# batd-htplus/intool-rag

Hardware: AMD Instinct MI355X
Metric: queries/sec, exact top-10 inner-product search, 1M x 1024-d fp32 index (higher is better)
Workload: dtype bf16 x bf16 -> f32 filter scan, f64 re-score of the f32 rows; 1 GPU; configs[1]: 1M x 1024-d synthetic unit vectors, brute-force inner-product top-10; rows=1000000, dim=1024, k=10, queries_per_pass=64, exchange=none, steps_in_flight=4, world=1, backend=none, allgather_payload_bytes_per_rank=0

## Files before the change

include/hiprag.h:

```cpp
#ifndef HIPRAG_H
#define HIPRAG_H

#include <stdint.h>

#ifdef __cplusplus
extern "C" {
#endif

#define HIPRAG_OK 0
#define HIPRAG_E_INVALID (-1)
#define HIPRAG_E_HIP (-2)
#define HIPRAG_E_HANDLE (-3)
#define HIPRAG_E_IO (-4)
#define HIPRAG_E_NOMEM (-5)
#define HIPRAG_E_UNSUPPORTED (-6)

#define HIPRAG_METRIC_IP 0
#define HIPRAG_METRIC_L2 1

int32_t hiprag_version(void);
const char* hiprag_last_error(void);
int32_t hiprag_device_count(int32_t* out_count);
int32_t hiprag_device_sync(int32_t device);
int32_t hiprag_scan_stream(int32_t device, void** out_stream);
// ... 54 lines not shown
    int32_t wide_env;
    int32_t n_cu;
    int32_t launch_env;
} hipidx_scan_shape_t;
typedef struct hipidx_scan_plan_t {
    int32_t run;
    int32_t wide;
    int32_t waves;
    int32_t ring;
    int32_t multi_pass;
    int32_t filter;
    int32_t ncls;
    int32_t qtile_image;
    int64_t lds_bytes;
    int32_t launch_queries;
    int32_t pipe_spare_cus;
    int64_t bytes_per_pass_ip;
    int64_t bytes_per_pass_l2;
} hipidx_scan_plan_t;
int32_t hiprag_scan_plan(const hipidx_scan_shape_t* shape, int32_t nq, int32_t k, int32_t cus, hipidx_scan_plan_t* out);
int32_t hipidx_scan_shape(uint64_t h, hipidx_scan_shape_t* out);
int32_t hiprag_wide_walk(int64_t nrt, int32_t ncol, int32_t cus, int32_t wg, int64_t cap, int64_t* out_row_tile,
                         int32_t* out_column, int64_t* out_pairs);
int32_t hipidx_gate_tail_dev(uint64_t h, int32_t slot, void* stream);
int32_t hipidx_reserve_search(uint64_t h, int32_t k);
int32_t hipidx_reserve_rows(uint64_t h, int64_t n_rows);
int32_t hipidx_reconstruct(uint64_t h, int64_t row, float* out_host);
int32_t hipidx_save(uint64_t h, const char* path);
int32_t hipidx_load(const char* path, int32_t device, uint64_t* out_handle);

typedef struct hipidx_stats {
    int64_t passes;
    int64_t queries;
    int64_t fallback_queries;
    int64_t bytes_per_pass;
    int64_t timed_passes;
    float avg_scan_ms;
    float avg_scan_wall_ms;
    float avg_scan_gap_ms;
    int64_t launches;
    int64_t roundb_queries;
    int64_t list_entries;
    int64_t ranked_entries;
    int64_t rescored_groups;
    int64_t wide_launches;
} hipidx_stats;
int32_t hipidx_get_stats(uint64_t h, hipidx_stats* out);
int32_t hipidx_enable_timing(uint64_t h, int32_t on);

int32_t hipivf_create(uint64_t rows_h, uint64_t centroids_h, const int64_t* list_offsets_host, const int64_t* orig_ids_host,
                      int32_t nlist, uint64_t* out_handle);
int32_t hipivf_destroy(uint64_t h);
int32_t hipivf_search_dev(uint64_t h, const float* q_dev, int32_t nq, int32_t k, int32_t nprobe, double* out_scores64_dev,
                          float* out_scores_dev, int64_t* out_ids_dev, void* stream);
int32_t hipivf_info(uint64_t h, int32_t* out_nlist, int64_t* out_stored_rows, int64_t* out_longest_list);
int32_t hipivf_search_batch_dev(uint64_t h, const float* q_dev, int32_t nq, int32_t k, int32_t nprobe,
                                double* out_scores64_dev, float* out_scores_dev, int64_t* out_ids_dev, void* stream);
int32_t hipivf_batch_info(uint64_t h, int64_t* out4);
int32_t hipivf_search_scoped_dev(uint64_t h, const float* q_dev, int32_t nq, int32_t k, int32_t nprobe,
                                 const int64_t* ranges_host, const int32_t* scope_offsets_host, int32_t n_scopes,
                                 const int32_t* scope_of_query_host, double* out_scores64_dev, float* out_scores_dev,
                                 int64_t* out_ids_dev, void* stream);
int32_t hipivf_search_scoped(uint64_t h, const float* q_host, int32_t nq, int32_t k, int32_t nprobe,
                             const int64_t* ranges_host, const int32_t* scope_offsets_host, int32_t n_scopes,
                             const int32_t* scope_of_query_host, double* out_scores64, float* out_scores, int64_t* out_ids);
int32_t hipivf_scoped_info(uint64_t h, int64_t* out4);
#define HIPIVF_PROBE_ANY   0
#define HIPIVF_PROBE_SCOPE 1
// ... 319 lines not shown
```

intool-rag_amd/csrc/dense_api.hip:

```cpp
#include <cstring>
#include <vector>

#include "common.h"
#include "dense_internal.h"

namespace hiprag {

Registry<DenseIndex>& reg()
{
    static Registry<DenseIndex> r;
    return r;
}

int32_t create_dense(int32_t d, int32_t metric, int32_t device, std::shared_ptr<DenseIndex>& out)
{
    HR_REQUIRE(d > 0, "d must be positive (got %d)", d);
    HR_REQUIRE(metric == HIPRAG_METRIC_IP || metric == HIPRAG_METRIC_L2, "unknown metric %d", metric);
    const int P = ((d + 127) / 128) * 16;
    if ((size_t)P * 1024 > 128 * 1024) {
        set_error("d=%d needs %d KiB of LDS for the query tile; the scan supports d <= 1024 (128 KiB, leaving 32 KiB per CU "
                  "for the tail kernels of earlier passes)", d, P);
        return HIPRAG_E_UNSUPPORTED;
    }
    auto ix = std::make_shared<DenseIndex>();
// ... 306 lines not shown

int32_t hipidx_get_stats(uint64_t h, hipidx_stats* out)
{
    GET_INDEX(h);
    HR_REQUIRE(out, "null out");
    HR_CHECK_HIP(hipDeviceSynchronize());
    unsigned long long fb = 0;
    HR_CHECK_HIP(hipMemcpy(&fb, ix->fallback_counter(), sizeof(fb), hipMemcpyDeviceToHost));
    out->passes = ix->passes;
    out->launches = ix->launches;
    out->queries = ix->queries;
    out->fallback_queries = (int64_t)fb;
    {
        unsigned long long rbq = 0;
        HR_CHECK_HIP(hipMemcpy(&rbq, ix->extend_counter(), sizeof(rbq), hipMemcpyDeviceToHost));
        out->roundb_queries = (int64_t)rbq;
        unsigned long long wc[3] = {0, 0, 0};
        HR_CHECK_HIP(hipMemcpy(wc, ix->work_counters(), sizeof(wc), hipMemcpyDeviceToHost));
        out->list_entries = (int64_t)wc[0];
        out->ranked_entries = (int64_t)wc[1];
        out->rescored_groups = (int64_t)wc[2];
    }
    out->wide_launches = ix->wide_launches;
    out->bytes_per_pass = bytes_per_pass(ix->shape(), ix->metric, ix->wide_launch(ix->launch_q));
    return ix->timing.summarise(ix->nblocks() > 0, out);
}

}
```

intool-rag_amd/csrc/dense_index.hip:

```cpp
#include <atomic>
#include <cfloat>
#include <cmath>
#include <chrono>
#include <cstring>
#include <vector>

#include "common.h"
#include "topk_device.h"
#include "dense_internal.h"

namespace hiprag {
namespace {

__global__ void retile_kernel(const float* __restrict__ src, int64_t row0, int64_t n, int d, int P,
                              float4* __restrict__ xb)
{
    const int64_t blk0 = row0 / kRowsPerBlock;
    const int64_t nblk = (row0 + n - 1) / kRowsPerBlock - blk0 + 1;
    const int64_t t = (int64_t)blockIdx.x * blockDim.x + threadIdx.x;
    if (t >= nblk * P * kPieceVec4) return;
    const int lane = (int)(t & 63);
    const int64_t pp = t >> 6;
    const int p = (int)(pp % P);
    const int64_t blk = blk0 + pp / P;
// ... 117 lines not shown
        if (pipe_done[i]) (void)hipEventDestroy(pipe_done[i]);
    }
    if (add_ev) (void)hipEventDestroy(add_ev);
    for (hipEvent_t e : sc.pin_ev) if (e) (void)hipEventDestroy(e);
}

int32_t DenseIndex::init()
{
    HR_CHECK_HIP(hipSetDevice(device));
    hipDeviceProp_t prop;
    HR_CHECK_HIP(hipGetDeviceProperties(&prop, device));
    n_cu = prop.multiProcessorCount > 0 ? prop.multiProcessorCount : 256;
    scan_cus = n_cu;
    if (const char* ms = getenv("HIPRAG_SCAN_MODE")) {
        if (!strcmp(ms, "bf16")) scan_mode = kScanBf16;
        else if (!strcmp(ms, "q64")) scan_mode = kScanQ64;
        else { set_error("HIPRAG_SCAN_MODE=%s: the scan has two operand modes, bf16 (default) and q64", ms); return HIPRAG_E_INVALID; }
    }
    if (const char* sw = getenv("HIPRAG_SCAN_WIDE")) {
        if (!strcmp(sw, "0")) scan_wide = 0;
        else if (!strcmp(sw, "1")) scan_wide = 1;
        else { set_error("HIPRAG_SCAN_WIDE=%s: 0 (never the wide scan kernel) or 1 (whenever a launch is eligible)", sw); return HIPRAG_E_INVALID; }
    }
    const char* lq = getenv("HIPRAG_LAUNCH_QUERIES");
    launch_env = lq ? atoi(lq) : 0;
    update_launch_q();
    int32_t rc = scalars.reserve(64);
    if (rc) return rc;
    if ((rc = started.reserve(256))) return rc;
    HR_CHECK_HIP(hipMemset(started.p, 0, 256));
    gate = started.as<unsigned long long>() + 16;
    HR_CHECK_HIP(hipMemset(scalars.p, 0, 64));
    HR_CHECK_HIP(hipStreamSynchronize(nullptr));
    return HIPRAG_OK;
}

int32_t DenseIndex::grow(int64_t need_blocks)
{
    if (need_blocks <= cap_blocks) return HIPRAG_OK;
    {
        const int32_t wrc = wait_adds_host();
        if (wrc) return wrc;
    }
    int64_t nc = cap_blocks == 0 ? need_blocks : std::max(need_blocks, cap_blocks + cap_blocks / 2);
    size_t xbytes = (size_t)nc * P * kPieceFloats * sizeof(float);
    size_t nbytes = (size_t)nc * kRowsPerBlock * sizeof(float);
// ... 174 lines not shown

template <int METRIC>
int32_t DenseIndex::scan_pass(const float* q_dev, int nq, int k, int slot, int cus, hipStream_t st)
{
    Workspace& w = ws[slot];
    const ScanPlan pl = plan(nq, k, cus);
    const bool use_ev = timing.bracket() && pl.run;
    w.seq = 0;
    if (pl.run) {
        if (w.dirty) HR_CHECK_HIP(hipMemsetAsync(w.state.p, 0, w.state.bytes, st));
        w.dirty = true;
        w.waves = pl.waves;
        ScanArgs sa;
        sa.xb = xb.as<float4>(); sa.xh = xh.p; sa.q = q_dev; sa.norms = norms.as<float>();
        sa.slots = st_slots(w); sa.thetac = st_thetac(w); sa.count = st_count(w);
        sa.list = w.list.as<Cand>();
        sa.nblocks = nblocks(); sa.ntotal = ntotal; sa.nq = nq; sa.d = d; sa.P = P;
        sa.filter = pl.filter ? 1 : 0;
        sa.ncls = pl.ncls;
        sa.stamps = timing.launch_stamps();
        w.seq = ++scan_seq;
        started_total += (unsigned long long)cus;
        sa.started = started.as<unsigned long long>(); sa.target = started_total; sa.seq = w.seq; sa.gate = gate;
        sa.qtile = nullptr;
        if (pl.qtile_image) {
            const int npass = (nq + kPassQ - 1) / kPassQ, per_pass = P * 64;
            hipLaunchKernelGGL(qtile_kernel, dim3((unsigned)((per_pass + 255) / 256), (unsigned)npass), dim3(256), 0, st, q_dev, nq, d,
                               P / 2, w.qtile.as<bf16x8>());
            sa.qtile = w.qtile.p;
        }
        const ScanKernel scan = scan_kernel_of<METRIC>(pl, scan_mode);
        if (pl.wide) ++wide_launches;
        { int32_t lrc = ensure_lds(reinterpret_cast<const void*>(scan), pl.lds_bytes); if (lrc) return lrc; }
        if (use_ev) HR_CHECK_HIP(hipEventRecord(timing.edge(0), st));
        hipLaunchKernelGGL(scan, dim3(cus), dim3(pl.waves * 64), pl.lds_bytes, st, sa);
        if (use_ev) HR_CHECK_HIP(hipEventRecord(timing.edge(1), st));
    }
    w.ev_idx = timing.note(use_ev, pl.run ? cus * w.waves : 0);
    HR_CHECK_HIP(hipGetLastError());
    passes += (nq + kPassQ - 1) / kPassQ;
    ++launches;
    queries += nq;
    return HIPRAG_OK;
}

template <int METRIC>
// ... 207 lines not shown
```

intool-rag_amd/csrc/dense_internal.h:

```cpp
#pragma once
#include <atomic>
#include <vector>

#include "common.h"
#include "dense_layout.h"
#include "dense_plan.h"

namespace hiprag {

struct GroupWorkspace {
    DevBuf tiles, len, offs, chunks, order, items, stat, ps, pi;
    i64 chunk = 0, chunks_n = 0;
};

struct ScanTiming {
    static constexpr int kEvRing = 512;
    static constexpr int kMaxScanWaves = 12;
    bool on = false;
    int every = 1;
    int64_t count = 0;
    std::vector<hipEvent_t> evs;
    DevBuf stamps;
    int n_cu = 0, wall_khz = 100000;
    std::vector<char> ev_set;
// ... 2 lines not shown
    ~ScanTiming() { for (hipEvent_t e : evs) (void)hipEventDestroy(e); }
    void enable(int n) { on = n != 0; every = std::max(1, n); count = 0; }
    int32_t ensure(int n_cu_, int device);
    int slot() const { return (int)(count % kEvRing); }
    bool bracket() const { return on && count % every == 0; }
    unsigned long long* launch_stamps() const
    {
        return on ? stamps.as<unsigned long long>() + (size_t)slot() * n_cu * kMaxScanWaves * 2 : nullptr;
    }
    hipEvent_t edge(int which) const { return evs[2 * slot() + which]; }
    int note(bool bracketed, int waves);
    int32_t summarise(bool have_rows, hipidx_stats* out) const;
};

struct DenseIndex {
    std::mutex mu;
    int device = 0;
    int d = 0, P = 0, metric = 0;
    int64_t ntotal = 0, cap_blocks = 0, id_base = 0;
    int n_cu = 256;
    int scan_cus = 256;
    ScanMode scan_mode = kScanBf16;
    int scan_wide = -1;
    DevBuf xb, xh, norms, scalars;
    struct Workspace {
        DevBuf list, state, flags, ek, ei;
        DevBuf qtile;
        int k = 0, q = 0;
        int64_t blocks = 0;
        int ev_idx = -1;
        bool dirty = false;
        int waves = 8;
        unsigned long long seq = 0;
    };
    static constexpr int kSlots = 8;
    Workspace ws[kSlots];
    DevBuf qbuf, o64, o32, oid;
    struct Scoped {
        static constexpr int kRing = 4;
        PinBuf pin[kRing];
        hipEvent_t pin_ev[kRing] = {nullptr, nullptr, nullptr, nullptr};
        bool pin_used[kRing] = {false, false, false, false};
        int pin_next = 0;
        DevBuf meta;
        GroupWorkspace gw;
        int32_t upload(const int64_t* img, size_t words, hipStream_t st);
    } sc;
    DevBuf score_stat;
    i64 score_pairs = 0;
    PinBuf pin_q, pin_o32, pin_oid, pin_flags;
    unsigned long long* gate = nullptr;
    DevBuf started;
    unsigned long long scan_seq = 0, started_total = 0;
    static constexpr int kFewQueries = 16;
    int launch_q = 256;
    int launch_env = 0;
    int64_t passes = 0, queries = 0, launches = 0, wide_launches = 0;
    ScanTiming timing;

    int64_t nblocks() const { return (ntotal + kRowsPerBlock - 1) / kRowsPerBlock; }
    unsigned* max_norm2_bits() { return scalars.as<unsigned>(); }
    unsigned* max_dx2_bits() { return scalars.as<unsigned>() + 1; }
    unsigned long long* fallback_counter() { return reinterpret_cast<unsigned long long*>(scalars.as<unsigned>() + 2); }
    unsigned long long* extend_counter() { return reinterpret_cast<unsigned long long*>(scalars.as<unsigned>() + 4); }
    unsigned long long* work_counters() { return reinterpret_cast<unsigned long long*>(scalars.as<unsigned>() + 6); }

    hipEvent_t add_ev = nullptr;
    bool add_pending = false;

    int32_t wait_adds_host()
    {
        if (add_pending) { HR_CHECK_HIP(hipEventSynchronize(add_ev)); add_pending = false; }
        return HIPRAG_OK;
    }
    int32_t wait_adds_stream(hipStream_t st)
    {
        if (add_pending) HR_CHECK_HIP(hipStreamWaitEvent(st, add_ev, 0));
        return HIPRAG_OK;
    }

    ~DenseIndex();
    int32_t init();
    int32_t grow(int64_t need_blocks);
    int32_t add_dev(const float* x_dev, int64_t n, hipStream_t st);
    int32_t add_host(const float* x, int64_t n);

    static constexpr size_t kRemoveBudget = (size_t)256 << 20;
    i64 rm_info[4] = {0, 0, 0, 0};
// ... 62 lines not shown
```

intool-rag_amd/csrc/dense_plan.h:

```cpp
#pragma once
#include <algorithm>
#include <cmath>
#include <cstddef>
#include <cstdint>

#include "../../include/hiprag.h"

namespace hiprag {

constexpr int kPassQ = 64;
constexpr int kMaxQ = 1024;
constexpr int kMaxKFast = 128;
constexpr int kClasses = 64;
constexpr int kNoFilterGroups = 1024;

constexpr int kStageHalf = 896;
constexpr int kThetaBack = 8;
constexpr int kCandBytes = 16;

constexpr int kWideBlocks = 8;
constexpr int kWideQTiles = 8;
constexpr int kWideKP = 2;
constexpr int kWideBufFrags = kWideBlocks * kWideKP * 64;
static_assert(kWideBlocks == kWideQTiles, "one slot size serves both rings");
// ... 85 lines not shown
    uint32_t rt, col;
};
constexpr uint32_t kWideNoTile = 0xFFFFFFFFu;
HIPRAG_HD inline WideWalk wide_walk(uint32_t nrt, uint32_t ncol, uint32_t G, uint32_t w)
{
    const uint32_t F = nrt / G, L = nrt - F * G;
    const uint32_t tail = F ? L * ncol : 0u;
    WideWalk W;
    W.ncol = ncol; W.G = G; W.w = w;
    W.full = (F ? F : 1u) * ncol;
    W.tail0 = F * G;
    W.npairs = w >= nrt ? 0u : W.full + (tail > w ? (tail - w + G - 1) / G : 0u);
    return W;
}
HIPRAG_HD inline WidePair wide_walk_pair(const WideWalk& W, uint32_t p)
{
    if (p >= W.npairs) return WidePair{kWideNoTile, 0u};
    const bool in_full = p < W.full;
    const uint32_t t = in_full ? p : W.w + (p - W.full) * W.G;
    const uint32_t r = t / W.ncol;
    return WidePair{in_full ? W.w + r * W.G : W.tail0 + r, t - r * W.ncol};
}

inline ScanPlan plan_scan(const ScanShape& s, int nq, int k, int cus)
{
    ScanPlan p;
    p.filter = filter_on(s);
    p.run = s.nblocks > 0 && k <= kMaxKFast;
    if (!p.run) return p;
    p.wide = wide_launch_on(s, nq, cus);
    p.waves = p.wide ? 8 : scan_waves(s, cus);
    p.multi_pass = nq > kPassQ;
    p.ring = p.wide ? 0 : (s.mode == kScanQ64 || (s.P / 2) % 16 == 0) ? 16 : 8;
    const int64_t bpw = ceil_div(s.nblocks, (int64_t)cus * p.waves);
    p.ncls = (int)std::max<int64_t>(1, std::min<int64_t>(kClasses, ceil_div(s.nblocks, bpw)));
    p.lds_bytes = p.wide ? kWideLds : (size_t)s.P * 1024 + (size_t)2 * kStageHalf * kCandBytes + 64 + (size_t)kThetaBack * 64 * 4;
    p.qtile_image = uses_qtile_images(s) && p.multi_pass;
    return p;
}

}
```

intool-rag_amd/csrc/dense_scan.h:

```cpp
#pragma once

constexpr int kCandCap = 4096;
constexpr int kPublish = 4;
constexpr int kDelay = 4;
constexpr int kAge = kPublish - 1 + kDelay;
constexpr int kRecompute = 2;

struct Cand {
    u64 key;
    float sec;
    u32 q;
};
static_assert(sizeof(Cand) == kCandBytes, "dense_plan.h sizes the staging area by kCandBytes");

struct ScanArgs {
    const float4* xb;
    const void* xh;
    const float* q;
    const void* qtile;
    const float* norms;
    u32* slots;
    u32* thetac;
    u32* count;
    Cand* list;
    int64_t nblocks;
    int64_t ntotal;
    int nq, d, P;
    int filter;
    int ncls;
    unsigned long long* stamps;
    unsigned long long* started;
    unsigned long long target, seq;
    unsigned long long* gate;
};

__host__ __device__ __forceinline__ int64_t scan_blocks_per_wave(int64_t nblocks, int64_t nwaves)
{
    return (nblocks + nwaves - 1) / nwaves;
}

__device__ __forceinline__ float tag_quad(float v, unsigned g) { return __uint_as_float((__float_as_uint(v) & ~3u) | g); }

template <int METRIC>
__device__ __forceinline__ float block_lane_top2(const f32x16& acc, const f32x4 (&nrm)[4], int64_t blk, int h, const ScanArgs& a,
                                                 float& second)
{
    float sc[16];
    if (METRIC == HIPRAG_METRIC_L2) {
#pragma unroll
        for (int g = 0; g < 4; ++g) {
            sc[4 * g + 0] = 2.f * acc[4 * g + 0] - nrm[g][0];
            sc[4 * g + 1] = 2.f * acc[4 * g + 1] - nrm[g][1];
            sc[4 * g + 2] = 2.f * acc[4 * g + 2] - nrm[g][2];
            sc[4 * g + 3] = 2.f * acc[4 * g + 3] - nrm[g][3];
        }
    } else {
// ... 595 lines not shown
```

intool-rag_amd/csrc/lib.cpp:

```cpp
#include "common.h"
#include "dense_plan.h"

#include <algorithm>
#include <cmath>
#include <map>
#include <memory>
#include <vector>

namespace hiprag {

static thread_local std::string g_last_error;

void set_error(const char* fmt, ...)
{
    char buf[1024];
    va_list ap;
    va_start(ap, fmt);
    vsnprintf(buf, sizeof(buf), fmt, ap);
    va_end(ap);
    g_last_error = buf;
}

static Registry<hipEvent_t>& events()
{
// ... 236 lines not shown
    clear_bm25_registry();
    clear_dense_registry();
    events().clear();
    leg_events().clear();
    scan_streams().clear();
    step_events().clear();
    return HIPRAG_OK;
}

int32_t hiprag_wide_walk(int64_t nrt, int32_t ncol, int32_t cus, int32_t wg, int64_t cap, int64_t* out_row_tile,
                         int32_t* out_column, int64_t* out_pairs)
{
    HR_REQUIRE(out_pairs, "null out");
    HR_REQUIRE(nrt >= 1 && nrt < ((int64_t)1 << 28) && ncol >= 1 && ncol <= kMaxQ / (kWideQTiles * 32) && cus >= 1 && wg >= 0 && wg < cus,
               "hiprag_wide_walk: 1 <= nrt < 2^28, 1 <= ncol <= %d, cus >= 1 and 0 <= wg < cus", kMaxQ / (kWideQTiles * 32));
    HR_REQUIRE(cap >= 0 && (cap == 0 || (out_row_tile && out_column)), "hiprag_wide_walk: cap > 0 needs both output arrays");
    const WideWalk W = wide_walk((uint32_t)nrt, (uint32_t)ncol, (uint32_t)cus, (uint32_t)wg);
    *out_pairs = W.npairs;
    for (uint32_t p = 0; p < W.npairs && (int64_t)p < cap; ++p) {
        const WidePair pr = wide_walk_pair(W, p);
        out_row_tile[p] = pr.rt;
        out_column[p] = (int32_t)pr.col;
    }
    return HIPRAG_OK;
}

int32_t hiprag_probe_read_gbps(int32_t device, int64_t bytes, int32_t reps, double* out_gbps)
{
    HR_REQUIRE(out_gbps && bytes >= (1 << 20) && reps > 0, "bad probe arguments");
    HR_CHECK_HIP(hipSetDevice(device));
    hipDeviceProp_t prop;
    HR_CHECK_HIP(hipGetDeviceProperties(&prop, device));
    const int ncu = prop.multiProcessorCount > 0 ? prop.multiProcessorCount : 256;
    const long long nblocks = bytes / 65536;
    const long long waves = (long long)ncu * 8;
    const int bpw = (int)((nblocks + waves - 1) / waves), passes = 4;
    void* x = nullptr;
    float* out = nullptr;
    HR_CHECK_HIP(hipMalloc(&x, (size_t)nblocks * 65536));
    hipError_t e = hipMalloc(&out, 64);
    if (e != hipSuccess) { (void)hipFree(x); HR_CHECK_HIP(e); }
    hipEvent_t e0 = nullptr, e1 = nullptr;
    float ms = 0.f;
    e = hipMemset(x, 0, (size_t)nblocks * 65536);
    if (e == hipSuccess) e = hipEventCreate(&e0);
    if (e == hipSuccess) e = hipEventCreate(&e1);
// ... 449 lines not shown
```

intool-rag_amd/csrc/scan_wide.h:

```cpp
#pragma once

constexpr int kWideQ = kWideQTiles * 32;
constexpr unsigned long long kWideWaitTicks = 20000ull;

constexpr int kWideBatch = 16;
constexpr int kWidePhaseT = kClasses / kWideBatch + 1;
constexpr int kWidePhaseA = kWidePhaseT + 1;
constexpr int kWidePhaseEvery = 2;

#define WIDE_DSR(dst, addr, off) asm volatile("ds_read_b128 %0, %1 offset:%2" : "=v"(dst) : "v"(addr), "n"(off) : "memory")
#define WIDE_LGKM1(n, x) asm volatile("s_waitcnt lgkmcnt(%[c])" : "+v"(x) : [c] "n"(n) : "memory")
#define WIDE_LGKM3(n, x, y, z) asm volatile("s_waitcnt lgkmcnt(%[c])" : "+v"(x), "+v"(y), "+v"(z) : [c] "n"(n) : "memory")

#define WIDE_BAR()                                \
    do {                                          \
        __builtin_amdgcn_sched_barrier(0);        \
        __builtin_amdgcn_s_barrier();             \
        __builtin_amdgcn_sched_barrier(0);        \
    } while (0)

struct WidePend {
    float f[4][2], s[4][2];
    u32 mn;
    int64_t rt;
    int unit;
    int phase;
};
struct WideFlight {
    u32 ld[kWideBatch];
    u32 tc;
    u32 pos0, pos1;
// ... 96 lines not shown
        P.mn = m;
    }
    if (P.phase == kWidePhaseA) {
        WIDE_WAIT2(YOUNGER, X.pos0, X.pos1);
        bool p0[4], p1[4];
        wide_test(a, P, bh, lane, P.mn, p0, p1);
        const int h = lane >> 5;
        const u32 q0 = (u32)(P.unit * 64 + (lane & 31)), q1 = q0 + 32;
        const int64_t blk0 = P.rt * kWideBlocks + 4 * bh;
        u32 pos0 = X.pos0, pos1 = X.pos1;
#pragma unroll
        for (int i = 0; i < 4; ++i) {
            const u32 gid = (u32)(2 * (blk0 + i) + h);
            if (p0[i]) {
                if (pos0 < (u32)kCandCap) a.list[(size_t)q0 * kCandCap + pos0] = Cand{pack_key(P.f[i][0], gid), P.s[i][0], q0};
                ++pos0;
            }
            if (p1[i]) {
                if (pos1 < (u32)kCandCap) a.list[(size_t)q1 * kCandCap + pos1] = Cand{pack_key(P.f[i][1], gid), P.s[i][1], q1};
                ++pos1;
            }
        }
    }
    P.phase = P.phase == kWidePhaseA ? 0 : P.phase + 1;
}

__device__ __forceinline__ void wide_drain(const ScanArgs& a, WidePend& P, int bh, int lane)
{
    while (P.phase) {
        WideFlight X;
        wide_issue(a, P, X, bh, lane);
        wide_land<true>(a, P, X, bh, lane);
    }
}

template <int METRIC>
__device__ __forceinline__ void wide_park(const ScanArgs& a, const f32x16 (&acc)[4][2], WidePend& P, int64_t rt, int unit, int bh, int lane)
{
    const int h = lane >> 5;
    const int64_t blk0 = rt * kWideBlocks + 4 * bh;
    if (blk0 >= a.nblocks) return;
    float pm0 = -INFINITY, pm1 = -INFINITY;
#pragma unroll
    for (int i = 0; i < 4; ++i) {
        const int64_t blk = blk0 + i;
        P.f[i][0] = P.f[i][1] = P.s[i][0] = P.s[i][1] = -FLT_MAX;
        if (blk < a.nblocks) {
            f32x4 nrm[4];
            if (METRIC == HIPRAG_METRIC_L2) {
#pragma unroll
                for (int g = 0; g < 4; ++g) nrm[g] = *reinterpret_cast<const f32x4*>(a.norms + blk * kRowsPerBlock + 8 * g + 4 * h);
            }
            P.f[i][0] = block_lane_top2<METRIC>(acc[i][0], nrm, blk, h, a, P.s[i][0]);
            P.f[i][1] = block_lane_top2<METRIC>(acc[i][1], nrm, blk, h, a, P.s[i][1]);
            pm0 = fmaxf(pm0, P.f[i][0]);
            pm1 = fmaxf(pm1, P.f[i][1]);
        }
    }
    {
        const float x0 = fmaxf(pm0, __shfl_xor(pm0, 32)), x1 = fmaxf(pm1, __shfl_xor(pm1, 32));
        const float v = lane < 32 ? x0 : x1;
        const int cls = (int)((2 * rt + bh) & (kClasses - 1));
        if (unit * 64 + lane < a.nq) atomicMax(a.slots + ((size_t)unit * kClasses + cls) * 64 + lane, ord32(v));
    }
    P.mn = 0xFFFFFFFFu;
    P.rt = rt;
    P.unit = unit;
    P.phase = 1;
}

template <int METRIC>
__global__ __launch_bounds__(512) void scan_wide_kernel(ScanArgs a)
{
    extern __shared__ float4 qs[];
    const int tid = threadIdx.x, lane = tid & 63;
    const int wave = __builtin_amdgcn_readfirstlane(tid >> 6);
    __builtin_amdgcn_s_setprio(3);
    const int64_t gw = (int64_t)blockIdx.x * 8 + wave;
    if (a.stamps && lane == 0) a.stamps[2 * gw] = wall_clock64();
    if (a.gate && tid == 0) {
        const unsigned long long was = __hip_atomic_fetch_add(a.started, 1ull, __ATOMIC_RELAXED, __HIP_MEMORY_SCOPE_AGENT);
        if (was + 1 == a.target) __hip_atomic_fetch_max(a.gate, a.seq, __ATOMIC_RELAXED, __HIP_MEMORY_SCOPE_AGENT);
    }
    const int P2 = a.P / 2;
    const int KS = P2 / kWideKP;
    const int nunits = (a.nq + 63) / 64;
    const int ncol = (a.nq + kWideQ - 1) / kWideQ;
    const int64_t nrt = (a.nblocks + kWideBlocks - 1) / kWideBlocks;
    const int bh = wave & 1, qp = wave >> 1;
    const bf16x8* xh = reinterpret_cast<const bf16x8*>(a.xh);
    const bf16x8* qimg = reinterpret_cast<const bf16x8*>(a.qtile);
// ... 4 lines not shown
    auto advance = [&](Cursor& c) -> bool {
        if (++c.ks < KS) return false;
        c.ks = 0;
        ++c.p;
        return true;
    };
    struct Stream { const bf16x8* p; u32 d; };
    auto row_stream = [&](int64_t rt) {
        const int64_t b0 = min(rt * kWideBlocks + (wave >> 1), a.nblocks - 1);
        const int64_t b1 = min(rt * kWideBlocks + (wave >> 1) + 4, a.nblocks - 1);
        return Stream{xh + ((size_t)b0 * P2 + (wave & 1)) * 64, (u32)(b1 - b0) * (u32)P2 * 64u};
    };
    auto query_stream = [&](int col) {
        const int t0 = min(col * kWideQTiles + (wave >> 1), 2 * nunits - 1);
        const int t1 = min(col * kWideQTiles + (wave >> 1) + 4, 2 * nunits - 1);
        return Stream{qimg + ((size_t)t0 * P2 + (wave & 1)) * 64, (u32)(t1 - t0) * (u32)P2 * 64u};
    };
    auto stage = [&](const Stream& S, int slot) {
        bf16x8* dst = lds + slot * kWideBufFrags + wave * 64;
        __builtin_amdgcn_global_load_lds((const void*)(S.p + lane), (scan_lds_ptr_t)dst, 16, 0, 0);
        __builtin_amdgcn_global_load_lds((const void*)(S.p + S.d + lane), (scan_lds_ptr_t)(dst + 8 * 64), 16, 0, 0);
    };

    f32x16 acc[4][2];
    WidePend P;
    P.phase = 0;
    if (W.npairs) {
        Cursor c{0, 0};
        uint32_t rt = blockIdx.x;
        int unit = qp;
        Cursor rc{0, 0}, qc{0, 0};
        Stream R = row_stream((int64_t)rt), Q = query_stream(0);
        auto next_rows = [&]() {
            R.p += kWideKP * 64;
            if (advance(rc)) R = row_stream((int64_t)wide_walk_pair(W, rc.p).rt);
        };
        auto next_queries = [&]() {
            Q.p += kWideKP * 64;
            if (advance(qc)) Q = query_stream((int)wide_walk_pair(W, qc.p).col);
        };
        int rslot = 0, qslot = 0;
        stage(R, 0); next_rows();
        stage(R, 1); next_rows();
        stage(Q, kWideRowRing + 0); next_queries();
        stage(R, 2); next_rows();
        stage(Q, kWideRowRing + 1); next_queries();
// ... 24 lines not shown
#define WIDE_PAIR(i, av, q0, q1)                                                                 \
                acc[i][0] = __builtin_amdgcn_mfma_f32_32x32x16_bf16(av, q0, acc[i][0], 0, 0, 0); \
                acc[i][1] = __builtin_amdgcn_mfma_f32_32x32x16_bf16(av, q1, acc[i][1], 0, 0, 0)
                WIDE_DSR(b0, B, 0); WIDE_DSR(b1, B, 2048);
                WIDE_DSR(a0, A, 0); WIDE_DSR(a1, A, 2048); WIDE_DSR(a2, A, 4096); WIDE_DSR(a3, A, 6144);
                WIDE_LGKM3(3, b0, b1, a0); WIDE_PAIR(0, a0, b0, b1);
                WIDE_DSR(c0, B, 1024);
                WIDE_LGKM1(3, a1); WIDE_PAIR(1, a1, b0, b1);
                WIDE_DSR(c1, B, 3072);
                WIDE_LGKM1(3, a2); WIDE_PAIR(2, a2, b0, b1);
                WIDE_DSR(a0, A, 1024);
                WIDE_LGKM1(3, a3); WIDE_PAIR(3, a3, b0, b1);
                WIDE_DSR(a1, A, 3072); WIDE_DSR(a2, A, 5120); WIDE_DSR(a3, A, 7168);
                WIDE_LGKM3(3, c0, c1, a0); WIDE_PAIR(0, a0, c0, c1); __builtin_amdgcn_sched_barrier(0);
                WIDE_LGKM1(2, a1); WIDE_PAIR(1, a1, c0, c1); __builtin_amdgcn_sched_barrier(0);
                WIDE_LGKM1(1, a2); WIDE_PAIR(2, a2, c0, c1); __builtin_amdgcn_sched_barrier(0);
                WIDE_LGKM1(0, a3); WIDE_PAIR(3, a3, c0, c1);
#undef WIDE_PAIR
            }
            __builtin_amdgcn_sched_barrier(0);
            if (pend) wide_land<false>(a, P, X, bh, lane_e);
            if (unit < nunits && c.ks == KS - 1) {
                wide_drain(a, P, bh, lane_e);
                wide_park<METRIC>(a, acc, P, (int64_t)rt, unit, bh, lane_e);
            }
            if (advance(c)) {
                const WidePair next = wide_walk_pair(W, c.p);
                rt = next.rt;
                unit = (int)next.col * (kWideQTiles / 2) + qp;
            }
            rslot = rslot == kWideRowRing - 1 ? 0 : rslot + 1;
            qslot = qslot == kWideQRing - 1 ? 0 : qslot + 1;
        } while (c.p < W.npairs);
    }
    asm volatile("s_waitcnt vmcnt(0)" ::: "memory");
    wide_drain(a, P, bh, lane);
    if (a.stamps && lane == 0) a.stamps[2 * gw + 1] = wall_clock64();
}
```

intool-rag_amd/hiprag/_native.py:

```python
from __future__ import annotations

import ctypes
import os
from ctypes import POINTER, c_char_p, c_double, c_float, c_int32, c_int64, c_uint32, c_uint64, c_void_p

_PKG_DIR = os.path.dirname(os.path.dirname(os.path.abspath(__file__)))
LIB_PATH = os.environ.get("HIPRAG_LIB", os.path.join(_PKG_DIR, "lib", "libhiprag.so"))

METRIC_IP = 0
METRIC_L2 = 1
PROBE_ANY = 0
PROBE_SCOPE = 1


class HipRagError(RuntimeError):

    def __init__(self, fn: str, code: int, msg: str):
        super().__init__(f"{fn} failed (status {code}): {msg}")
        self.code = code


class HipIdxStats(ctypes.Structure):
    _fields_ = [("passes", c_int64), ("queries", c_int64), ("fallback_queries", c_int64),
                ("bytes_per_pass", c_int64), ("timed_passes", c_int64), ("avg_scan_ms", c_float),
                ("avg_scan_wall_ms", c_float), ("avg_scan_gap_ms", c_float), ("launches", c_int64), ("roundb_queries", c_int64),
                ("list_entries", c_int64), ("ranked_entries", c_int64), ("rescored_groups", c_int64),
                ("wide_launches", c_int64)]


class HipIdxScanShape(ctypes.Structure):
    _fields_ = [("nblocks", c_int64), ("P", c_int32), ("mode", c_int32), ("wide_env", c_int32), ("n_cu", c_int32),
                ("launch_env", c_int32)]


class HipIdxScanPlan(ctypes.Structure):
    _fields_ = [("run", c_int32), ("wide", c_int32), ("waves", c_int32), ("ring", c_int32), ("multi_pass", c_int32),
                ("filter", c_int32), ("ncls", c_int32), ("qtile_image", c_int32), ("lds_bytes", c_int64),
                ("launch_queries", c_int32), ("pipe_spare_cus", c_int32), ("bytes_per_pass_ip", c_int64),
                ("bytes_per_pass_l2", c_int64)]


class HipEncShape(ctypes.Structure):
    _fields_ = [("hidden", c_int32), ("ffn", c_int32), ("n_cu", c_int32), ("small_rows", c_int32), ("use256", c_int32)]


class HipEncPlan(ctypes.Structure):
    _fields_ = [("T", c_int32), ("M", c_int32), ("path", c_int32), ("osplit", c_int32), ("dsplit", c_int32), ("fsplit", c_int32),
                ("head_split", c_int32), ("pre_bytes", c_int64)]


# ... 49 lines not shown
    "hipidx_search_scoped_dev": [c_uint64, c_void_p, c_int32, c_int32, c_void_p, c_void_p, c_int32, c_void_p, c_void_p, c_void_p,
                                 c_void_p, c_void_p],
    "hipidx_search_scoped": [c_uint64, c_void_p, c_int32, c_int32, c_void_p, c_void_p, c_int32, c_void_p, c_void_p, c_void_p,
                             c_void_p],
    "hipidx_scoped_info": [c_uint64, c_void_p],
    "hiprag_scope_plan": [c_void_p, c_void_p, c_int32, c_void_p, c_int32, c_int64, c_int32, c_int32, c_void_p, c_void_p, c_int64],
    "hipidx_score_ids_dev": [c_uint64, c_void_p, c_int32, c_void_p, c_int32, c_void_p, c_void_p, c_void_p],
    "hipidx_score_ids": [c_uint64, c_void_p, c_int32, c_void_p, c_int32, c_void_p, c_void_p],
    "hipidx_score_info": [c_uint64, c_void_p],
    "hipidx_remove_ranges": [c_uint64, c_void_p, c_int32],
    "hipidx_remove_info": [c_uint64, c_void_p],
    "hipidx_row_bounds": [c_uint64, c_void_p],
    "hipidx_search_begin_dev": [c_uint64, c_void_p, c_int32, c_int32, c_int32, c_void_p],
    "hipidx_search_finish_dev": [c_uint64, c_void_p, c_int32, c_int32, c_int32, c_void_p, c_void_p, c_void_p, c_void_p],
    "hipidx_pass_queries": [c_uint64, i32p],
    "hipidx_launch_queries": [c_uint64, i32p],
    "hipidx_set_spare_cus": [c_uint64, c_int32],
    "hipidx_get_spare_cus": [c_uint64, c_void_p],
    "hipidx_pipe_spare_cus": [c_uint64, c_void_p],
    "hipidx_gate_tail_dev": [c_uint64, c_int32, c_void_p],
    "hiprag_scan_plan": [POINTER(HipIdxScanShape), c_int32, c_int32, c_int32, POINTER(HipIdxScanPlan)],
    "hipidx_scan_shape": [c_uint64, POINTER(HipIdxScanShape)],
    "hiprag_wide_walk": [c_int64, c_int32, c_int32, c_int32, c_int64, c_void_p, c_void_p, c_void_p],
    "hiprag_compaction_plan": [c_void_p, c_int64, c_void_p, c_int32, c_void_p, c_void_p],
    "hipidx_reserve_search": [c_uint64, c_int32],
    "hipidx_reserve_rows": [c_uint64, c_int64],
    "hipidx_reconstruct": [c_uint64, c_int64, c_void_p],
    "hipidx_save": [c_uint64, c_char_p],
    "hipidx_load": [c_char_p, c_int32, u64p],
    "hipidx_get_stats": [c_uint64, POINTER(HipIdxStats)],
    "hipidx_enable_timing": [c_uint64, c_int32],
    "hipivf_create": [c_uint64, c_uint64, c_void_p, c_void_p, c_int32, u64p],
    "hipivf_destroy": [c_uint64],
    "hipivf_search_dev": [c_uint64, c_void_p, c_int32, c_int32, c_int32, c_void_p, c_void_p, c_void_p, c_void_p],
    "hipivf_info": [c_uint64, i32p, i64p, i64p],
    "hipivf_search_batch_dev": [c_uint64, c_void_p, c_int32, c_int32, c_int32, c_void_p, c_void_p, c_void_p, c_void_p],
    "hipivf_batch_info": [c_uint64, c_void_p],
    "hipivf_search_scoped_dev": [c_uint64, c_void_p, c_int32, c_int32, c_int32, c_void_p, c_void_p, c_int32, c_void_p, c_void_p,
                                 c_void_p, c_void_p, c_void_p],
    "hipivf_search_scoped": [c_uint64, c_void_p, c_int32, c_int32, c_int32, c_void_p, c_void_p, c_int32, c_void_p, c_void_p,
                             c_void_p, c_void_p],
    "hipivf_scoped_info": [c_uint64, c_void_p],
    "hipivf_search_scoped_probe_dev": [c_uint64, c_void_p, c_int32, c_int32, c_int32, c_int32, c_void_p, c_void_p, c_int32, c_void_p,
                                       c_void_p, c_void_p, c_void_p, c_void_p],
    "hipivf_search_scoped_probe": [c_uint64, c_void_p, c_int32, c_int32, c_int32, c_int32, c_void_p, c_void_p, c_int32, c_void_p,
                                   c_void_p, c_void_p, c_void_p],
# ... 174 lines not shown
```

intool-rag_amd/hiprag/index.py:

```python
from __future__ import annotations

import ctypes
from typing import Optional, Tuple

import numpy as np

from . import _native as nat
from ._native import METRIC_IP, METRIC_L2, HipRagError

_METRICS = {"ip": METRIC_IP, "l2": METRIC_L2, METRIC_IP: METRIC_IP, METRIC_L2: METRIC_L2}


def _host_f32(a, cols: Optional[int] = None) -> np.ndarray:
    a = np.ascontiguousarray(a, dtype=np.float32)
    if a.ndim == 1:
        a = a[None, :]
    if a.ndim != 2 or (cols is not None and a.shape[1] != cols):
        raise ValueError(f"expected a [n,{cols}] float32 array, got shape {a.shape}")
    return a


def scan_plan(shape: "nat.HipIdxScanShape", nq: int, k: int, cus: int) -> "nat.HipIdxScanPlan":
    p = nat.HipIdxScanPlan()
    nat.call("hiprag_scan_plan", ctypes.byref(shape), int(nq), int(k), int(cus), ctypes.byref(p))
    return p


def wide_walk(nrt: int, ncol: int, cus: int, wg: int) -> Tuple[np.ndarray, np.ndarray]:
    n = ctypes.c_int64()
    nat.call("hiprag_wide_walk", int(nrt), int(ncol), int(cus), int(wg), 0, None, None, ctypes.byref(n))
    rts, cols = np.empty(n.value, np.int64), np.empty(n.value, np.int32)
    nat.call("hiprag_wide_walk", int(nrt), int(ncol), int(cus), int(wg), n.value, rts.ctypes.data, cols.ctypes.data, ctypes.byref(n))
    return rts, cols


class HipFlatIndex:
    def __init__(self, d: int, metric="l2", device: int = 0, _handle: Optional[int] = None):
        self.device = int(device)
        if _handle is None:
            h = ctypes.c_uint64()
            nat.call("hipidx_create", int(d), _METRICS[metric], self.device, ctypes.byref(h))
            self._h = h.value
        else:
            self._h = _handle
        self.d = int(d)
        self.metric = _METRICS[metric]

    def close(self) -> None:
        if getattr(self, "_h", None):
            try:
                nat.call("hipidx_destroy", self._h)
            finally:
                self._h = None

    def __del__(self):
        try:
# ... 308 lines not shown
```

Baseline: 410,300 queries/s.

## Fold wide-scan unit bounds only on a staggered subset of tiles

The wide scan kernel used to recompute each query unit's threshold (theta fold, a multi-phase reduction over class slots) after every parked tile. Now it folds only in the first few tiles and then in one tile out of N (default 8), with the offset staggered per workgroup and wave. Non-folding tiles skip straight to the tail phase or pass through idle phases. A final fold runs at the end if the last tile skipped it, and a fold counter is added to stats. This cuts the per-tile reduction work and atomics, but thresholds go stale between folds, so pruning is looser and more candidates may pass the filter.

Result: faster. 425,900 queries/s (median of 6 runs) (+3.8%).

```diff
diff --git a/include/hiprag.h b/include/hiprag.h
--- a/include/hiprag.h
+++ b/include/hiprag.h
@@ -100,6 +100,8 @@
 int32_t hipidx_scan_shape(uint64_t h, hipidx_scan_shape_t* out);
 int32_t hiprag_wide_walk(int64_t nrt, int32_t ncol, int32_t cus, int32_t wg, int64_t cap, int64_t* out_row_tile,
                          int32_t* out_column, int64_t* out_pairs);
+int32_t hiprag_wide_fold(int64_t p0, int64_t n, int32_t wg, int32_t wave, int32_t every, uint8_t* out_fold, int32_t* out_first,
+                         int32_t* out_default);
 int32_t hipidx_gate_tail_dev(uint64_t h, int32_t slot, void* stream);
 int32_t hipidx_reserve_search(uint64_t h, int32_t k);
 int32_t hipidx_reserve_rows(uint64_t h, int64_t n_rows);
@@ -122,6 +124,7 @@
     int64_t ranked_entries;
     int64_t rescored_groups;
     int64_t wide_launches;
+    int64_t wide_theta_folds;
 } hipidx_stats;
 int32_t hipidx_get_stats(uint64_t h, hipidx_stats* out);
 int32_t hipidx_enable_timing(uint64_t h, int32_t on);
diff --git a/intool-rag_amd/csrc/dense_api.hip b/intool-rag_amd/csrc/dense_api.hip
--- a/intool-rag_amd/csrc/dense_api.hip
+++ b/intool-rag_amd/csrc/dense_api.hip
@@ -352,6 +352,11 @@
         out->rescored_groups = (int64_t)wc[2];
     }
     out->wide_launches = ix->wide_launches;
+    {
+        unsigned long long folds = 0;
+        HR_CHECK_HIP(hipMemcpy(&folds, ix->fold_counter(), sizeof(folds), hipMemcpyDeviceToHost));
+        out->wide_theta_folds = (int64_t)folds;
+    }
     out->bytes_per_pass = bytes_per_pass(ix->shape(), ix->metric, ix->wide_launch(ix->launch_q));
     return ix->timing.summarise(ix->nblocks() > 0, out);
 }
diff --git a/intool-rag_amd/csrc/dense_index.hip b/intool-rag_amd/csrc/dense_index.hip
--- a/intool-rag_amd/csrc/dense_index.hip
+++ b/intool-rag_amd/csrc/dense_index.hip
@@ -163,6 +163,15 @@
         else if (!strcmp(sw, "1")) scan_wide = 1;
         else { set_error("HIPRAG_SCAN_WIDE=%s: 0 (never the wide scan kernel) or 1 (whenever a launch is eligible)", sw); return HIPRAG_E_INVALID; }
     }
+    if (const char* fe = getenv("HIPRAG_WIDE_FOLD_EVERY")) {
+        char* end = nullptr;
+        const long n = strtol(fe, &end, 10);
+        if (end == fe || *end || !wide_fold_every_ok(n)) {
+            set_error("HIPRAG_WIDE_FOLD_EVERY=%s: a power of two in 1..%d (the wide scan recomputes a unit's bound in one tile out of so many; 1 = in every tile)", fe, kWideFoldMax);
+            return HIPRAG_E_INVALID;
+        }
+        wide_fold_every = (int)n;
+    }
     const char* lq = getenv("HIPRAG_LAUNCH_QUERIES");
     launch_env = lq ? atoi(lq) : 0;
     update_launch_q();
@@ -383,6 +392,7 @@
         w.seq = ++scan_seq;
         started_total += (unsigned long long)cus;
         sa.started = started.as<unsigned long long>(); sa.target = started_total; sa.seq = w.seq; sa.gate = gate;
+        sa.fold_every = wide_fold_every; sa.folds = fold_counter();
         sa.qtile = nullptr;
         if (pl.qtile_image) {
             const int npass = (nq + kPassQ - 1) / kPassQ, per_pass = P * 64;
diff --git a/intool-rag_amd/csrc/dense_internal.h b/intool-rag_amd/csrc/dense_internal.h
--- a/intool-rag_amd/csrc/dense_internal.h
+++ b/intool-rag_amd/csrc/dense_internal.h
@@ -48,6 +48,7 @@
     int scan_cus = 256;
     ScanMode scan_mode = kScanBf16;
     int scan_wide = -1;
+    int wide_fold_every = kWideFoldEvery;
     DevBuf xb, xh, norms, scalars;
     struct Workspace {
         DevBuf list, state, flags, ek, ei;
@@ -90,6 +91,7 @@
     unsigned long long* fallback_counter() { return reinterpret_cast<unsigned long long*>(scalars.as<unsigned>() + 2); }
     unsigned long long* extend_counter() { return reinterpret_cast<unsigned long long*>(scalars.as<unsigned>() + 4); }
     unsigned long long* work_counters() { return reinterpret_cast<unsigned long long*>(scalars.as<unsigned>() + 6); }
+    unsigned long long* fold_counter() { return reinterpret_cast<unsigned long long*>(scalars.as<unsigned>() + 12); }
 
     hipEvent_t add_ev = nullptr;
     bool add_pending = false;
diff --git a/intool-rag_amd/csrc/dense_plan.h b/intool-rag_amd/csrc/dense_plan.h
--- a/intool-rag_amd/csrc/dense_plan.h
+++ b/intool-rag_amd/csrc/dense_plan.h
@@ -131,6 +131,21 @@
     return WidePair{in_full ? W.w + r * W.G : W.tail0 + r, t - r * W.ncol};
 }
 
+constexpr int kWideFoldFirst = 4;
+constexpr int kWideFoldMax = 64;
+constexpr int kWideFoldEvery = 8;
+inline bool wide_fold_every_ok(int64_t N) { return N >= 1 && N <= kWideFoldMax && (N & (N - 1)) == 0; }
+HIPRAG_HD inline uint32_t wide_fold_key(uint32_t wg, uint32_t wave, uint32_t N)
+{
+    const uint32_t bh = wave & 1u, qp = wave >> 1;
+    return ((2u * wg + bh + qp) & (uint32_t)(kWideFoldMax - 1)) | ((N - 1u) << 8);
+}
+HIPRAG_HD inline bool wide_fold_at(uint32_t p, uint32_t key)
+{
+    return p < (uint32_t)kWideFoldFirst || ((p + (key & 0xFFu)) & (key >> 8)) == 0u;
+}
+HIPRAG_HD inline bool wide_fold(uint32_t p, uint32_t wg, uint32_t wave, uint32_t N) { return wide_fold_at(p, wide_fold_key(wg, wave, N)); }
+
 inline ScanPlan plan_scan(const ScanShape& s, int nq, int k, int cus)
 {
     ScanPlan p;
diff --git a/intool-rag_amd/csrc/dense_scan.h b/intool-rag_amd/csrc/dense_scan.h
--- a/intool-rag_amd/csrc/dense_scan.h
+++ b/intool-rag_amd/csrc/dense_scan.h
@@ -32,6 +32,8 @@
     unsigned long long* started;
     unsigned long long target, seq;
     unsigned long long* gate;
+    int fold_every;
+    unsigned long long* folds;
 };
 
 __host__ __device__ __forceinline__ int64_t scan_blocks_per_wave(int64_t nblocks, int64_t nwaves)
diff --git a/intool-rag_amd/csrc/lib.cpp b/intool-rag_amd/csrc/lib.cpp
--- a/intool-rag_amd/csrc/lib.cpp
+++ b/intool-rag_amd/csrc/lib.cpp
@@ -282,6 +282,18 @@
         out_row_tile[p] = pr.rt;
         out_column[p] = (int32_t)pr.col;
     }
+    return HIPRAG_OK;
+}
+
+int32_t hiprag_wide_fold(int64_t p0, int64_t n, int32_t wg, int32_t wave, int32_t every, uint8_t* out_fold, int32_t* out_first,
+                         int32_t* out_default)
+{
+    HR_REQUIRE(p0 >= 0 && n >= 0 && p0 + n <= ((int64_t)1 << 31) && wg >= 0 && wg < (1 << 28) && wave >= 0 && wave < 8 && wide_fold_every_ok(every),
+               "hiprag_wide_fold: 0 <= p0, p0 + n <= 2^31, 0 <= wg < 2^28, 0 <= wave < 8, every a power of two in 1..%d", kWideFoldMax);
+    HR_REQUIRE(n == 0 || out_fold, "hiprag_wide_fold: n > 0 needs the output array");
+    for (int64_t i = 0; i < n; ++i) out_fold[i] = wide_fold((uint32_t)(p0 + i), (uint32_t)wg, (uint32_t)wave, (uint32_t)every) ? 1 : 0;
+    if (out_first) *out_first = kWideFoldFirst;
+    if (out_default) *out_default = kWideFoldEvery;
     return HIPRAG_OK;
 }
 
diff --git a/intool-rag_amd/csrc/scan_wide.h b/intool-rag_amd/csrc/scan_wide.h
--- a/intool-rag_amd/csrc/scan_wide.h
+++ b/intool-rag_amd/csrc/scan_wide.h
@@ -6,7 +6,10 @@
 constexpr int kWideBatch = 16;
 constexpr int kWidePhaseT = kClasses / kWideBatch + 1;
 constexpr int kWidePhaseA = kWidePhaseT + 1;
+constexpr int kWidePhaseIdle = kWidePhaseA + 1;
+constexpr int kWidePhaseIdleLast = kWidePhaseIdle + kClasses / kWideBatch - 1;
 constexpr int kWidePhaseEvery = 2;
+constexpr bool kWideFoldLate = true;
 
 #define WIDE_DSR(dst, addr, off) asm volatile("ds_read_b128 %0, %1 offset:%2" : "=v"(dst) : "v"(addr), "n"(off) : "memory")
 #define WIDE_LGKM1(n, x) asm volatile("s_waitcnt lgkmcnt(%[c])" : "+v"(x) : [c] "n"(n) : "memory")
@@ -149,11 +152,12 @@
             }
         }
     }
-    P.phase = P.phase == kWidePhaseA ? 0 : P.phase + 1;
+    P.phase = P.phase == kWidePhaseA ? 0 : P.phase == kWidePhaseIdleLast ? kWidePhaseT : P.phase + 1;
 }
 
 __device__ __forceinline__ void wide_drain(const ScanArgs& a, WidePend& P, int bh, int lane)
 {
+    if (P.phase >= kWidePhaseIdle) P.phase = kWidePhaseT;
     while (P.phase) {
         WideFlight X;
         wide_issue(a, P, X, bh, lane);
@@ -162,7 +166,7 @@
 }
 
 template <int METRIC>
-__device__ __forceinline__ void wide_park(const ScanArgs& a, const f32x16 (&acc)[4][2], WidePend& P, int64_t rt, int unit, int bh, int lane)
+__device__ __forceinline__ void wide_park(const ScanArgs& a, const f32x16 (&acc)[4][2], WidePend& P, int64_t rt, int unit, bool fold, int bh, int lane)
 {
     const int h = lane >> 5;
     const int64_t blk0 = rt * kWideBlocks + 4 * bh;
@@ -190,10 +194,10 @@
         const int cls = (int)((2 * rt + bh) & (kClasses - 1));
         if (unit * 64 + lane < a.nq) atomicMax(a.slots + ((size_t)unit * kClasses + cls) * 64 + lane, ord32(v));
     }
-    P.mn = 0xFFFFFFFFu;
+    P.mn = fold ? 0xFFFFFFFFu : 0u;
     P.rt = rt;
     P.unit = unit;
-    P.phase = 1;
+    P.phase = fold ? 1 : kWideFoldLate ? kWidePhaseIdle : kWidePhaseT;
 }
 
 template <int METRIC>
@@ -244,6 +248,8 @@
         __builtin_amdgcn_global_load_lds((const void*)(S.p + S.d + lane), (scan_lds_ptr_t)(dst + 8 * 64), 16, 0, 0);
     };
 
+    u32 fold_key = wide_fold_key(blockIdx.x, (uint32_t)wave, (uint32_t)a.fold_every);
+    asm volatile("" : "+v"(fold_key));
     f32x16 acc[4][2];
     WidePend P;
     P.phase = 0;
@@ -314,7 +320,8 @@
             if (pend) wide_land<false>(a, P, X, bh, lane_e);
             if (unit < nunits && c.ks == KS - 1) {
                 wide_drain(a, P, bh, lane_e);
-                wide_park<METRIC>(a, acc, P, (int64_t)rt, unit, bh, lane_e);
+                asm volatile("" : "+v"(fold_key));
+                wide_park<METRIC>(a, acc, P, (int64_t)rt, unit, wide_fold_at(c.p, (uint32_t)__builtin_amdgcn_readfirstlane((int)fold_key)), bh, lane_e);
             }
             if (advance(c)) {
                 const WidePair next = wide_walk_pair(W, c.p);
@@ -327,5 +334,29 @@
     }
     asm volatile("s_waitcnt vmcnt(0)" ::: "memory");
     wide_drain(a, P, bh, lane);
+    if (a.fold_every > 1) {
+        const uint32_t key = (uint32_t)__builtin_amdgcn_readfirstlane((int)fold_key);
+        for (uint32_t p = W.npairs; p-- > 0;) {
+            const WidePair pr = wide_walk_pair(W, p);
+            const int u = (int)pr.col * (kWideQTiles / 2) + qp;
+            if (u < nunits && (int64_t)pr.rt * kWideBlocks + 4 * bh < a.nblocks) {
+                if (!wide_fold_at(p, key)) (void)wide_theta_fresh(a, u, lane, u * 64 + lane < a.nq);
+                break;
+            }
+        }
+    }
     if (a.stamps && lane == 0) a.stamps[2 * gw + 1] = wall_clock64();
-}
+    if (wave == 0) {
+        const uint32_t wv = (uint32_t)lane & 7u;
+        const uint32_t key = wide_fold_key(blockIdx.x, wv, (uint32_t)a.fold_every);
+        u32 nf = 0;
+        for (uint32_t p = (uint32_t)lane >> 3; p < W.npairs; p += 8) {
+            const WidePair pr = wide_walk_pair(W, p);
+            const bool parked = (int)pr.col * (kWideQTiles / 2) + (int)(wv >> 1) < nunits && (int64_t)pr.rt * kWideBlocks + 4 * (int)(wv & 1u) < a.nblocks;
+            nf += parked && wide_fold_at(p, key) ? 1u : 0u;
+        }
+#pragma unroll
+        for (int off = 32; off >= 1; off >>= 1) nf += (u32)__shfl_xor((int)nf, off);
+        if (lane == 0 && nf) atomicAdd(a.folds, (unsigned long long)nf);
+    }
+}
diff --git a/intool-rag_amd/hiprag/_native.py b/intool-rag_amd/hiprag/_native.py
--- a/intool-rag_amd/hiprag/_native.py
+++ b/intool-rag_amd/hiprag/_native.py
@@ -25,7 +25,7 @@
                 ("bytes_per_pass", c_int64), ("timed_passes", c_int64), ("avg_scan_ms", c_float),
                 ("avg_scan_wall_ms", c_float), ("avg_scan_gap_ms", c_float), ("launches", c_int64), ("roundb_queries", c_int64),
                 ("list_entries", c_int64), ("ranked_entries", c_int64), ("rescored_groups", c_int64),
-                ("wide_launches", c_int64)]
+                ("wide_launches", c_int64), ("wide_theta_folds", c_int64)]
 
 
 class HipIdxScanShape(ctypes.Structure):
@@ -121,6 +121,7 @@
     "hiprag_scan_plan": [POINTER(HipIdxScanShape), c_int32, c_int32, c_int32, POINTER(HipIdxScanPlan)],
     "hipidx_scan_shape": [c_uint64, POINTER(HipIdxScanShape)],
     "hiprag_wide_walk": [c_int64, c_int32, c_int32, c_int32, c_int64, c_void_p, c_void_p, c_void_p],
+    "hiprag_wide_fold": [c_int64, c_int64, c_int32, c_int32, c_int32, c_void_p, c_void_p, c_void_p],
     "hiprag_compaction_plan": [c_void_p, c_int64, c_void_p, c_int32, c_void_p, c_void_p],
     "hipidx_reserve_search": [c_uint64, c_int32],
     "hipidx_reserve_rows": [c_uint64, c_int64],
diff --git a/intool-rag_amd/hiprag/index.py b/intool-rag_amd/hiprag/index.py
--- a/intool-rag_amd/hiprag/index.py
+++ b/intool-rag_amd/hiprag/index.py
@@ -32,6 +32,18 @@
     rts, cols = np.empty(n.value, np.int64), np.empty(n.value, np.int32)
     nat.call("hiprag_wide_walk", int(nrt), int(ncol), int(cus), int(wg), n.value, rts.ctypes.data, cols.ctypes.data, ctypes.byref(n))
     return rts, cols
+
+
+def wide_fold(p0: int, n: int, wg: int, wave: int, every: int) -> np.ndarray:
+    out = np.empty(int(n), np.uint8)
+    nat.call("hiprag_wide_fold", int(p0), int(n), int(wg), int(wave), int(every), out.ctypes.data, None, None)
+    return out.astype(bool)
+
+
+def wide_fold_constants() -> Tuple[int, int]:
+    first, default = ctypes.c_int32(), ctypes.c_int32()
+    nat.call("hiprag_wide_fold", 0, 0, 0, 0, 1, None, ctypes.byref(first), ctypes.byref(default))
+    return first.value, default.value
 
 
 class HipFlatIndex:
```
